# BattleZips/BattleZips-Halo2

Hardware: AMD Instinct MI355X
Metric: complete proofs per second (synthesis + create_proof), BoardCircuit, k=14, IPA/Pasta (higher is better)
Workload: dtype u32x8 (255-bit modular integer, Montgomery)

## Files before the change

### battlezips-halo2_amd/csrc/ntt.hip

```cpp
#include <cstdlib>
#include <cstring>
#include <vector>

#include "ntt_common.cuh"

namespace bzh {

template <class P>
void launch_ntt_pass_wave(const NttPassArgs& aa, unsigned tiles, unsigned nb, hipStream_t stream);
extern template void launch_ntt_pass_wave<FpParams>(const NttPassArgs&, unsigned, unsigned, hipStream_t);
extern template void launch_ntt_pass_wave<FqParams>(const NttPassArgs&, unsigned, unsigned, hipStream_t);
extern template void launch_ntt_pass_wave<BnFrParams>(const NttPassArgs&, unsigned, unsigned, hipStream_t);

template <class P, int C, bool FIRST>
__device__ __forceinline__ void stage_group(uint4* tile, const NttPassArgs& g, int s0, int items, int tid) {
    constexpr int E = 1 << C;
    const int r = g.r, logW = g.logW, W = 1 << logW;
    const int ngroups = items >> C;
    const int stride = 1 << (s0 + logW);
    for (int gi = tid; gi < ngroups; gi += kNttThreads) {
        const int col = gi & (W - 1), gg = gi >> logW;
        const int lo = gg & ((1 << s0) - 1), hi = gg >> s0;
        const int base = ((((hi << C) << s0) | lo) << logW) + col;
        Fe<P> x[E];
#pragma unroll
        for (int m = 0; m < E; m++) x[m] = tile_get<P>(tile, base + m * stride);
#pragma unroll
        for (int t = 0; t < C; t++) {
            const int sh = r - 1 - (s0 + t);
#pragma unroll
            for (int b = 0; b < E / 2; b++) {
                const int jm = b & ((1 << t) - 1), top = ((b >> t) << (t + 1)) + jm, bot = top + (1 << t);
                Fe<P> v = x[bot];
                if (!(FIRST && jm == 0)) {
                    const int j = FIRST ? jm : (lo | (jm << s0));
                    v = fe_mul(v, fe_load<P>(g.sub_tw + ((size_t)j << sh) * 8));
                }
                x[bot] = fe_sub(x[top], v);
                x[top] = fe_add(x[top], v);
            }
            __builtin_amdgcn_sched_barrier(0);
        }
#pragma unroll
        for (int m = 0; m < E; m++) tile_put(tile, base + m * stride, x[m]);
    }
}

template <class P>
__global__ void __launch_bounds__(kNttThreads) __attribute__((amdgpu_waves_per_eu(2))) k_ntt_pass(NttPassArgs g) {
    __shared__ __align__(16) uint4 tile[2 * kTileElems];
    const int tid = threadIdx.x, T = kNttThreads;
    const int r = g.r, R = 1 << r, logW = g.logW, W = 1 << logW;
    const size_t N = (size_t)1 << g.log_n;
    const uint32_t* vin = g.src + (size_t)blockIdx.y * N * 8;
    uint32_t* vec = g.dst + (size_t)blockIdx.y * N * 8;
    const size_t tile_id = blockIdx.x;
    const int items = R << logW;

    if (!g.last) {
        const size_t B = (size_t)1 << g.logB;
        const size_t tiles_per_a = B >> logW;
        const size_t a = tile_id / tiles_per_a, j0 = (tile_id - a * tiles_per_a) << logW;
        const uint32_t* base = vin + ((a << (r + g.logB)) + j0) * 8;
        if (g.nz) {
            const uint32_t* sv = g.src + (size_t)blockIdx.y * (N >> g.nz) * 8 + j0 * 8;
            const int live = items >> g.nz;
            for (int it = tid; it < live; it += T) {
                const int col = it & (W - 1), row = it >> logW;
                Fe<P> v = fe_load<P>(sv + ((size_t)row * B + col) * 8);
                if (g.pre_lo) v = fe_mul(v, pow_table<P>(g.pre_lo, g.pre_hi, g.h, (size_t)row * B + j0 + col));
                if (g.cube_pre) {
                    const unsigned c3 = (unsigned)(((size_t)row * B + j0 + col) % 3);
                    if (c3) v = fe_mul(v, cube_const<P>(g, c3));
                }
                const int p0 = (int)(bitrev((uint32_t)row, r) << logW) + col;
                for (int m = 0; m < (1 << g.nz); m++) tile_put(tile, p0 + (m << logW), v);
            }
        } else
        for (int it = tid; it < items; it += T) {
            const int col = it & (W - 1), row = it >> logW;
            Fe<P> v = fe_load<P>(base + ((size_t)row * B + col) * 8);
            if (g.pre_lo) v = fe_mul(v, pow_table<P>(g.pre_lo, g.pre_hi, g.h, (size_t)row * B + j0 + col));
            if (g.cube_pre) {
                const unsigned c3 = (unsigned)(((size_t)row * B + j0 + col) % 3);
                if (c3) v = fe_mul(v, cube_const<P>(g, c3));
            }
            tile_put(tile, (int)(bitrev((uint32_t)row, r) << logW) + col, v);
        }
    } else {
        for (int it = tid; it < items; it += T) {
            const int rr = it & (R - 1), i = it >> r;
            size_t d = (tile_id << logW) + i, a = 0;
            for (int q = 0; q < g.nprev; q++) {
                a = (a << g.prev_bits[q]) | (d & (((size_t)1 << g.prev_bits[q]) - 1));
                d >>= g.prev_bits[q];
            }
            Fe<P> v = fe_load<P>(vin + ((a << r) + rr) * 8);
            if (g.pre_lo) v = fe_mul(v, pow_table<P>(g.pre_lo, g.pre_hi, g.h, (size_t)rr));
            if (g.cube_pre && (rr % 3)) v = fe_mul(v, cube_const<P>(g, (unsigned)(rr % 3)));
            tile_put(tile, (int)(bitrev((uint32_t)rr, r) << logW) + i, v);
        }
    }
    {
        int s0 = g.nz ? g.nz : (r < 3 ? r : 3);
        if (!g.nz) {
            __syncthreads();
            switch (s0) {
                case 1: stage_group<P, 1, true>(tile, g, 0, items, tid); break;
                case 2: stage_group<P, 2, true>(tile, g, 0, items, tid); break;
                default: stage_group<P, 3, true>(tile, g, 0, items, tid); break;
            }
        }
        int ngr = (r - s0 + 2) / 3;
        for (; ngr > 0; ngr--) {
            const int c = (r - s0 + ngr - 1) / ngr;
            __syncthreads();
            switch (c) {
                case 1: stage_group<P, 1, false>(tile, g, s0, items, tid); break;
                case 2: stage_group<P, 2, false>(tile, g, s0, items, tid); break;
                default: stage_group<P, 3, false>(tile, g, s0, items, tid); break;
            }
            s0 += c;
        }
    }
    __syncthreads();
    if (!g.last) {
        const size_t B = (size_t)1 << g.logB;
        const size_t tiles_per_a = B >> logW;
        const size_t a = tile_id / tiles_per_a, j0 = (tile_id - a * tiles_per_a) << logW;
        uint32_t* base = vec + ((a << (r + g.logB)) + j0) * 8;
        for (int it = tid; it < items; it += T) {
            const int col = it & (W - 1), row = it >> logW;
            Fe<P> v = tile_get<P>(tile, it);
            if (g.tw_direct) {
                v = fe_mul(v, fe_load<P>(g.tw_direct + ((size_t)row * B + j0 + col) * 8));
            } else {
                const size_t e = ((size_t)row * (j0 + col)) << g.logA;
                if (e || g.tw_always) v = fe_mul(v, pow_table<P>(g.tw_lo, g.tw_hi, g.h, e));
            }
            fe_store(base + ((size_t)row * B + col) * 8, v);
        }
    } else {
        for (int it = tid; it < items; it += T) {
            const int i = it & (W - 1), kr = it >> logW;
            Fe<P> v = tile_get<P>(tile, it);
            const size_t k = ((size_t)kr << g.logA) + (tile_id << logW) + i;
            if (g.post_lo) v = fe_mul(v, pow_table<P>(g.post_lo, g.post_hi, g.h, k));
            if (g.cube_post) v = fe_mul(v, cube_const<P>(g, (unsigned)(k % 3)));
            ntt_store_out<P>(g, vec, (size_t)blockIdx.y, (size_t)1 << g.log_n, k, v);
        }
    }
}

struct NttDomain {
    int field;
    unsigned log_n;
    int inverse;
    int has_shift;
    uint32_t omega[8];
    uint32_t shift[8];
    int h;
    uint32_t* d_tables = nullptr;
    size_t off_tw_lo, off_tw_hi, off_sc_lo, off_sc_hi;
    size_t off_tw_hi_scaled;
    int shift_is_cube;
    uint32_t cube[3][8];
    size_t off_sub[12];
    size_t off_direct[4];
};

struct NttCache {
    std::vector<NttDomain> doms;
};
static std::mutex g_cache_mu;
static std::vector<std::pair<bzh_ctx*, NttCache*>> g_caches;

static NttCache* cache_for(bzh_ctx* ctx) {
    std::lock_guard<std::mutex> lk(g_cache_mu);
    for (auto& p : g_caches)
        if (p.first == ctx) return p.second;
    g_caches.emplace_back(ctx, new NttCache());
    return g_caches.back().second;
}
void ntt_cache_drop(bzh_ctx* ctx) {
    std::lock_guard<std::mutex> lk(g_cache_mu);
    for (size_t i = 0; i < g_caches.size(); i++)
        if (g_caches[i].first == ctx) {
            for (auto& d : g_caches[i].second->doms)
                if (d.d_tables) (void)hipFree(d.d_tables);
            delete g_caches[i].second;
            g_caches.erase(g_caches.begin() + i);
            return;
        }
}

template <class P>
static void fill_pows(std::vector<uint32_t>& out, size_t off, const Fe<P>& base, const Fe<P>& first, size_t count) {
    Fe<P> acc = first;
    for (size_t i = 0; i < count; i++) {
        for (int k = 0; k < 8; k++) out[off + i * 8 + k] = acc.l[k];
        acc = fe_mul(acc, base);
    }
}
template <class P>
static Fe<P> pow2k(Fe<P> x, int k) {
    for (int i = 0; i < k; i++) x = fe_sqr(x);
    return x;
}

static int plan_passes(unsigned log_n, int* bits) {
    if (log_n <= 11) {
        bits[0] = (int)log_n;
        return 1;
    }
    const int np = (int)((log_n + 8) / 9);
    const int base = (int)log_n / np, extra = (int)log_n % np;
    for (int i = 0; i < np; i++) bits[i] = base + (i < extra ? 1 : 0);
    return np;
}
static constexpr unsigned kDirectTwiddleMaxLog = 20;

template <class P>
static int build_domain(bzh_ctx* ctx, NttDomain& d, const Fe<P>& omega_m, const Fe<P>* shift_m) {
    const unsigned k = d.log_n;
    const size_t N = (size_t)1 << k;
    d.h = (int)((k + 1) / 2);
    const size_t nlo = (size_t)1 << d.h, nhi = (size_t)1 << (k - d.h);
    Fe<P> w = d.inverse ? fe_inv(omega_m) : omega_m;
    size_t words = 0;
    d.off_tw_lo = words; words += nlo * 8;
    d.off_tw_hi = words; words += nhi * 8;
    d.off_sc_lo = words; words += nlo * 8;
    d.off_sc_hi = words; words += nhi * 8;
    d.off_tw_hi_scaled = words; words += nhi * 8;
    for (int rb = 1; rb <= 11; rb++) {
        d.off_sub[rb] = words;
        if ((unsigned)rb <= k) words += ((size_t)1 << (rb - 1)) * 8;
    }
    int bits[5];
    const int np = plan_passes(k, bits);
    for (int p = 0; p < 4; p++) d.off_direct[p] = 0;
    if (np >= 2 && k <= kDirectTwiddleMaxLog) {
        int logA = 0;
        for (int p = 0; p + 1 < np; p++) {
            d.off_direct[p] = words;
            words += (N >> logA) * 8;
            logA += bits[p];
        }
    }
    std::vector<uint32_t> host(words, 0u);
    fill_pows<P>(host, d.off_tw_lo, w, fe_one<P>(), nlo);
    fill_pows<P>(host, d.off_tw_hi, pow2k(w, d.h), fe_one<P>(), nhi);
    Fe<P> sbase = fe_one<P>(), first_hi = fe_one<P>();
    if (d.has_shift) sbase = d.inverse ? fe_inv(*shift_m) : *shift_m;
    if (d.inverse) {
        Fe<P> nn = fe_zero<P>();
        nn.l[0] = (uint32_t)(N & 0xffffffffu);
        nn.l[1] = (uint32_t)((uint64_t)N >> 32);
        first_hi = fe_inv(fe_to_mont(nn));
    }
    fill_pows<P>(host, d.off_sc_lo, sbase, fe_one<P>(), nlo);
    fill_pows<P>(host, d.off_sc_hi, pow2k(sbase, d.h), first_hi, nhi);
    fill_pows<P>(host, d.off_tw_hi_scaled, pow2k(w, d.h), first_hi, nhi);
    {
        const Fe<P> s2 = fe_sqr(sbase), s3 = fe_mul(s2, sbase);
        d.shift_is_cube = d.has_shift && fe_eq(s3, fe_one<P>()) && !fe_eq(sbase, fe_one<P>());
        const Fe<P> c0 = first_hi, c1 = fe_mul(first_hi, sbase), c2 = fe_mul(first_hi, s2);
        for (int q = 0; q < 8; q++) {
            d.cube[0][q] = c0.l[q];
            d.cube[1][q] = c1.l[q];
            d.cube[2][q] = c2.l[q];
        }
    }
    for (int rb = 1; rb <= 11 && (unsigned)rb <= k; rb++) {
        Fe<P> wr = pow2k(w, (int)k - rb);
        fill_pows<P>(host, d.off_sub[rb], wr, fe_one<P>(), (size_t)1 << (rb - 1));
    }
    if (d.off_direct[0]) {
        int logA = 0;
        for (int p = 0; p + 1 < np; p++) {
            const size_t R = (size_t)1 << bits[p], B = N >> (logA + bits[p]);
            const Fe<P> wa = pow2k(w, logA);
            const Fe<P> first = (p == 0 && d.inverse && !d.has_shift) ? first_hi : fe_one<P>();
            Fe<P> wrow = fe_one<P>();
            for (size_t row = 0; row < R; row++) {
                fill_pows<P>(host, d.off_direct[p] + row * B * 8, wrow, first, B);
                wrow = fe_mul(wrow, wa);
            }
            logA += bits[p];
        }
    }
    BZH_HIP_TRY(ctx, hipMalloc((void**)&d.d_tables, words * 4));
    BZH_HIP_TRY(ctx, hipMemcpyAsync(d.d_tables, host.data(), words * 4, hipMemcpyHostToDevice, ctx->stream));
    BZH_HIP_TRY(ctx, hipStreamSynchronize(ctx->stream));
    return BZH_OK;
}

template <class P>
static int ntt_run_t(bzh_ctx* ctx, uint32_t* d_data, unsigned log_n, size_t batch, const uint64_t* omega,
                     const uint64_t* coset_shift, int inverse, int form, const uint32_t* d_src = nullptr, unsigned src_log = 0,
                     uint32_t* d_out29 = nullptr) {
    if (log_n == 0) return d_out29 ? BZH_E_ARG : BZH_OK;
    Fe<P> w, sh = fe_one<P>();
    for (int i = 0; i < 4; i++) {
        w.l[2 * i] = (uint32_t)omega[i];
        w.l[2 * i + 1] = (uint32_t)(omega[i] >> 32);
        if (coset_shift) {
            sh.l[2 * i] = (uint32_t)coset_shift[i];
            sh.l[2 * i + 1] = (uint32_t)(coset_shift[i] >> 32);
        }
    }
    if (form == BZH_FORM_CANONICAL) {
        w = fe_to_mont(w);
        if (coset_shift) sh = fe_to_mont(sh);
    }
    NttCache* cache = cache_for(ctx);
    NttDomain* dom = nullptr;
    for (auto& d : cache->doms) {
        if (d.field == P::id && d.log_n == log_n && d.inverse == (inverse != 0) && d.has_shift == (coset_shift != nullptr) &&
            memcmp(d.omega, w.l, 32) == 0 && (!coset_shift || memcmp(d.shift, sh.l, 32) == 0)) {
            dom = &d;
            break;
        }
    }
    if (!dom) {
        NttDomain d;
        d.field = P::id;
        d.log_n = log_n;
        d.inverse = inverse != 0;
        d.has_shift = coset_shift != nullptr;
        memcpy(d.omega, w.l, 32);
        memcpy(d.shift, sh.l, 32);
        int rc = build_domain<P>(ctx, d, w, coset_shift ? &sh : nullptr);
        if (rc) return rc;
        cache->doms.push_back(d);
        dom = &cache->doms.back();
    }
    const size_t total = batch << log_n;
    if (form == BZH_FORM_CANONICAL) {
        int rc = field_convert(ctx, P::id, d_data, total, 1);
        if (rc) return rc;
    }
    int bits[5];
    const int np = plan_passes(log_n, bits);
    int nz = 0;
    if (d_src) {
        if (src_log > log_n || form != BZH_FORM_MONTGOMERY) return BZH_E_ARG;
        nz = (int)(log_n - src_log);
        if ((np < 2 || nz > bits[0] || nz == 0) && !d_data) return BZH_E_ARG;
        if (np < 2 || nz > bits[0] || nz == 0) {
            BZH_HIP_TRY(ctx, hipMemsetAsync(d_data, 0, total * 32, ctx->stream));
            BZH_HIP_TRY(ctx, hipMemcpy2DAsync(d_data, ((size_t)32) << log_n, d_src, ((size_t)32) << src_log, ((size_t)32) << src_log, batch,
                                              hipMemcpyDeviceToDevice, ctx->stream));
            nz = 0;
            d_src = nullptr;
        }
    }
    uint32_t* d_scratch = nullptr;
    if (np >= 2) {
        void* sp = nullptr;
        int rc = ws_ensure(ctx, 0, total * 32, &sp);
        if (rc) return rc;
        d_scratch = (uint32_t*)sp;
    }
    const bool pre = (!inverse && coset_shift);
    const bool post = (inverse != 0);
    int logA = 0;
    for (int p = 0; p < np; p++) {
        NttPassArgs a;
        a.src = (p == 0) ? (nz ? d_src : d_data) : d_scratch;
        a.nz = (p == 0) ? nz : 0;
        a.dst = (p == np - 1) ? d_data : d_scratch;
        a.log_n = log_n;
        a.r = bits[p];
        a.logA = logA;
        a.logB = (int)log_n - logA - bits[p];
        a.last = (p == np - 1);
        int logW = 11 - a.r;
        if (!a.last && logW > a.logB) logW = a.logB;
        if (a.last && logW > logA) logW = logA;
        a.logW = logW;
        a.nprev = p;
        for (int q = 0; q < 4; q++) a.prev_bits[q] = q < p ? bits[q] : 0;
        a.sub_tw = dom->d_tables + dom->off_sub[a.r];
        a.tw_lo = dom->d_tables + dom->off_tw_lo;
        a.tw_hi = dom->d_tables + dom->off_tw_hi;
        a.tw_direct = (p + 1 < np && dom->off_direct[p]) ? dom->d_tables + dom->off_direct[p] : nullptr;
        a.h = dom->h;
        a.pre_lo = (pre && p == 0) ? dom->d_tables + dom->off_sc_lo : nullptr;
        a.pre_hi = dom->d_tables + dom->off_sc_hi;
        a.post_lo = (post && a.last) ? dom->d_tables + dom->off_sc_lo : nullptr;
        a.post_hi = dom->d_tables + dom->off_sc_hi;
        a.cube_pre = a.cube_post = a.tw_always = 0;
        a.dst29 = nullptr;
        memcpy(a.cube, dom->cube, sizeof(a.cube));
        if (pre && dom->shift_is_cube) {
            if (p == 0) a.cube_pre = 1;
            a.pre_lo = nullptr;
        }
        if (post) {
            if (coset_shift && dom->shift_is_cube) {
                a.post_lo = nullptr;
                a.cube_post = a.last ? 1 : 0;
            } else if (!coset_shift) {
                a.post_lo = nullptr;
                if (np == 1) {
                    a.cube_post = 1;
                } else if (p == 0) {
                    a.tw_hi = dom->d_tables + dom->off_tw_hi_scaled;
                    a.tw_always = 1;
                }
            }
        }
        const size_t tiles = ((size_t)1 << log_n) >> (a.r + logW);
        {
            ScopedTimer t(ctx, BZH_T_NTT);
            if (ctx->profiling && p == 0)
                ctx->alg_bytes[BZH_T_NTT] += (32.0 + (nz ? 32.0 / (double)(1 << nz) : 32.0)) * (double)batch * (double)((size_t)1 << log_n);
            for (size_t b0 = 0; b0 < batch; b0 += 65535) {
                size_t nb = batch - b0 < 65535 ? batch - b0 : 65535;
                NttPassArgs aa = a;
                aa.src = a.src + (b0 << (log_n - (unsigned)a.nz)) * 8;
                aa.dst = a.dst ? a.dst + (b0 << log_n) * 8 : nullptr;
                aa.dst29 = (a.last && d_out29) ? d_out29 + (b0 << log_n) * 9 : nullptr;
                static const bool lds_only = getenv("BZH_NTT_LDS") != nullptr;
                const dim3 grid((unsigned)tiles, (unsigned)nb), blk(kNttThreads);
                constexpr bool wave_ok = P::id != BZH_FIELD_BN254_FQ;
                if (wave_ok && !lds_only && a.r >= 6 && a.r <= 9 && logW == 11 - a.r && a.nz <= 3) {
                    if constexpr (wave_ok) launch_ntt_pass_wave<P>(aa, (unsigned)tiles, (unsigned)nb, ctx->stream);
                } else {
                    hipLaunchKernelGGL((k_ntt_pass<P>), grid, blk, 0, ctx->stream, aa);
                }
            }
        }
        BZH_HIP_TRY(ctx, hipGetLastError());
        logA += bits[p];
    }
    if (form == BZH_FORM_CANONICAL) {
        int rc = field_convert(ctx, P::id, d_data, total, 0);
        if (rc) return rc;
    }
    return BZH_OK;
}

template <class P>
__global__ void __launch_bounds__(256) k_field_convert(uint32_t* data, size_t count, int to_mont) {
    size_t gid = blockIdx.x * (size_t)blockDim.x + threadIdx.x;
    if (gid >= count) return;
    Fe<P> v = fe_load<P>(data + gid * 8);
    fe_store(data + gid * 8, to_mont ? fe_to_mont(v) : fe_from_mont(v));
}

int field_convert(bzh_ctx* ctx, int field, uint32_t* d, size_t count, int to_mont) {
    if (!count) return BZH_OK;
    dim3 grid((unsigned)((count + 255) / 256)), block(256);
    switch (field) {
        case BZH_FIELD_FP: hipLaunchKernelGGL((k_field_convert<FpParams>), grid, block, 0, ctx->stream, d, count, to_mont); break;
        case BZH_FIELD_FQ: hipLaunchKernelGGL((k_field_convert<FqParams>), grid, block, 0, ctx->stream, d, count, to_mont); break;
        case BZH_FIELD_BN254_FR: hipLaunchKernelGGL((k_field_convert<BnFrParams>), grid, block, 0, ctx->stream, d, count, to_mont); break;
        case BZH_FIELD_BN254_FQ: hipLaunchKernelGGL((k_field_convert<BnFqParams>), grid, block, 0, ctx->stream, d, count, to_mont); break;
        default: return BZH_E_ARG;
    }
    BZH_HIP_TRY(ctx, hipGetLastError());
    return BZH_OK;
}

int ntt_run(bzh_ctx* ctx, int field, uint32_t* d_data, unsigned log_n, size_t batch, const uint64_t* omega,
            const uint64_t* coset_shift, int inverse, int form) {
    switch (field) {
        case BZH_FIELD_FP: return ntt_run_t<FpParams>(ctx, d_data, log_n, batch, omega, coset_shift, inverse, form);
        case BZH_FIELD_FQ: return ntt_run_t<FqParams>(ctx, d_data, log_n, batch, omega, coset_shift, inverse, form);
        case BZH_FIELD_BN254_FR: return ntt_run_t<BnFrParams>(ctx, d_data, log_n, batch, omega, coset_shift, inverse, form);
        case BZH_FIELD_BN254_FQ: return ntt_run_t<BnFqParams>(ctx, d_data, log_n, batch, omega, coset_shift, inverse, form);
    }
    return BZH_E_ARG;
}

int ntt_run_padded(bzh_ctx* ctx, int field, uint32_t* d_dst, const uint32_t* d_src, unsigned src_log, unsigned log_n, size_t batch,
                   const uint64_t* omega, const uint64_t* coset_shift, uint32_t* d_out29) {
    const int f = BZH_FORM_MONTGOMERY;
    if (d_out29 && field != BZH_FIELD_FP && field != BZH_FIELD_FQ) return BZH_E_ARG;
    switch (field) {
        case BZH_FIELD_FP: return ntt_run_t<FpParams>(ctx, d_dst, log_n, batch, omega, coset_shift, 0, f, d_src, src_log, d_out29);
        case BZH_FIELD_FQ: return ntt_run_t<FqParams>(ctx, d_dst, log_n, batch, omega, coset_shift, 0, f, d_src, src_log, d_out29);
        case BZH_FIELD_BN254_FR: return ntt_run_t<BnFrParams>(ctx, d_dst, log_n, batch, omega, coset_shift, 0, f, d_src, src_log);
        case BZH_FIELD_BN254_FQ: return ntt_run_t<BnFqParams>(ctx, d_dst, log_n, batch, omega, coset_shift, 0, f, d_src, src_log);
    }
    return BZH_E_ARG;
}

}
```

### battlezips-halo2_amd/csrc/ntt_common.cuh

```cuda
#pragma once
#include "ctx.hpp"
#include "field.cuh"
#include "fe29.cuh"

namespace bzh {

static constexpr int kTileElems = 2048;
static constexpr int kNttThreads = 256;

struct NttPassArgs {
    const uint32_t* src;
    uint32_t* dst;
    unsigned log_n;
    int r;
    int logA;
    int logB;
    int logW;
    int last;
    int nprev;
    int prev_bits[4];
    const uint32_t* sub_tw;
    const uint32_t* tw_lo;
    const uint32_t* tw_hi;
    const uint32_t* tw_direct;
    int h;
    const uint32_t* pre_lo;
    const uint32_t* pre_hi;
    const uint32_t* post_lo;
    const uint32_t* post_hi;
    int cube_pre;
    int cube_post;
    int tw_always;
    int nz;
    uint32_t cube[3][8];
    uint32_t* dst29;
};
template <class P>
__device__ __forceinline__ void ntt_store_out(const NttPassArgs& g, uint32_t* vec, size_t vec_index, size_t N, size_t k, const Fe<P>& v) {
    if constexpr (fe29_supported<P>()) {
        if (g.dst29) {
            fe29_store_planes<P>(g.dst29 + vec_index * 9 * N, k, N, fe29_from_sat_reduced(v));
            return;
        }
    }
    fe_store(vec + k * 8, v);
}

template <class P>
__device__ __forceinline__ Fe<P> tile_get(const uint4* t, int idx) {
    uint4 a = t[idx], b = t[kTileElems + idx];
    Fe<P> r;
    r.l[0] = a.x; r.l[1] = a.y; r.l[2] = a.z; r.l[3] = a.w;
    r.l[4] = b.x; r.l[5] = b.y; r.l[6] = b.z; r.l[7] = b.w;
    return r;
}
template <class P>
__device__ __forceinline__ void tile_put(uint4* t, int idx, const Fe<P>& v) {
    t[idx] = make_uint4(v.l[0], v.l[1], v.l[2], v.l[3]);
    t[kTileElems + idx] = make_uint4(v.l[4], v.l[5], v.l[6], v.l[7]);
}
template <class P>
__device__ __forceinline__ Fe<P> pow_table(const uint32_t* lo, const uint32_t* hi, int h, size_t e) {
    Fe<P> a = fe_load<P>(lo + (e & (((size_t)1 << h) - 1)) * 8);
    Fe<P> b = fe_load<P>(hi + (e >> h) * 8);
    return fe_mul(a, b);
}
template <class P>
__device__ __forceinline__ Fe<P> cube_const(const NttPassArgs& g, unsigned i) {
    Fe<P> r;
#pragma unroll
    for (int k = 0; k < 8; k++) r.l[k] = i == 0 ? g.cube[0][k] : (i == 1 ? g.cube[1][k] : g.cube[2][k]);
    return r;
}
__device__ __forceinline__ uint32_t bitrev(uint32_t x, int bits) { return bits ? (__brev(x) >> (32 - bits)) : 0u; }


}
```

### battlezips-halo2_amd/csrc/ntt_wave.cuh

```cuda
#pragma once
#include "ntt_common.cuh"

namespace bzh {

template <int LB>
__device__ __forceinline__ void lane_swap_u32(uint32_t& lo, uint32_t& hi, bool lane_bit) {
    if constexpr (LB == 5) {
        auto r = __builtin_amdgcn_permlane32_swap(lo, hi, false, false);
        lo = r[0], hi = r[1];
    } else if constexpr (LB == 4) {
        auto r = __builtin_amdgcn_permlane16_swap(lo, hi, false, false);
        lo = r[0], hi = r[1];
    } else if constexpr (LB == 3) {
        const uint32_t nh = (uint32_t)__builtin_amdgcn_update_dpp((int)hi, (int)lo, 0x108 , 0xf, 0x3, false);
        const uint32_t nl = (uint32_t)__builtin_amdgcn_update_dpp((int)lo, (int)hi, 0x118 , 0xf, 0xc, false);
        lo = nl, hi = nh;
    } else if constexpr (LB == 2) {
        const uint32_t nh = (uint32_t)__builtin_amdgcn_update_dpp((int)hi, (int)lo, 0x104 , 0xf, 0x5, false);
        const uint32_t nl = (uint32_t)__builtin_amdgcn_update_dpp((int)lo, (int)hi, 0x114 , 0xf, 0xa, false);
        lo = nl, hi = nh;
    } else {
        const uint32_t send = lane_bit ? lo : hi;
        const uint32_t recv = (uint32_t)__builtin_amdgcn_mov_dpp((int)send, LB == 1 ? 0x4e  : 0xb1 ,
                                                                 0xf, 0xf, false);
        lo = lane_bit ? recv : lo;
        hi = lane_bit ? hi : recv;
    }
}
template <class P, int RB, int LB>
__device__ __forceinline__ void lane_swap(Fe<P> (&x)[8], int lane) {
    const bool lb = (lane >> LB) & 1;
#pragma unroll
    for (int m = 0; m < 8; m++) {
        if (m & (1 << RB)) continue;
#pragma unroll
        for (int q = 0; q < 8; q++) lane_swap_u32<LB>(x[m].l[q], x[m | (1 << RB)].l[q], lb);
    }
}
template <class P, int RB, class Tw>
__device__ __forceinline__ void reg_stage(Fe<P> (&x)[8], Tw tw) {
#pragma unroll
    for (int m = 0; m < 8; m++) {
        if (m & (1 << RB)) continue;
        Fe<P> v = x[m | (1 << RB)];
        const uint32_t* t = tw(m);
        if (t) v = fe_mul(v, fe_load<P>(t));
        x[m | (1 << RB)] = fe_sub(x[m], v);
        x[m] = fe_add(x[m], v);
    }
    __builtin_amdgcn_sched_barrier(0);
}

template <class P, int R, bool LAST>
__global__ void __launch_bounds__(kNttThreads) k_ntt_pass_wave(NttPassArgs g) {
    static_assert(R >= 6 && R <= 9, "three register bits + three to six lane bits");
    constexpr int RL = R - 3, CL = 6 - RL, N2 = RL - 3;
    const int lane = threadIdx.x & 63, wave = threadIdx.x >> 6;
    const int logW = g.logW;
    const int col = (wave << CL) | (lane & ((1 << CL) - 1));
    const int lr = lane >> CL;
    const size_t N = (size_t)1 << g.log_n;
    const uint32_t* vin = g.src + (size_t)blockIdx.y * N * 8;
    uint32_t* vec = g.dst + (size_t)blockIdx.y * N * 8;
    const size_t tile_id = blockIdx.x;
    const size_t B = (size_t)1 << g.logB;
    const size_t tiles_per_a = LAST ? 1 : (B >> logW);
    const size_t a_idx = LAST ? 0 : tile_id / tiles_per_a, j0 = LAST ? 0 : ((tile_id - a_idx * tiles_per_a) << logW);

    Fe<P> x[8];
    if (!LAST) {
        const uint32_t* base = g.nz ? g.src + (size_t)blockIdx.y * (N >> g.nz) * 8 + j0 * 8 : vin + ((a_idx << (R + g.logB)) + j0) * 8;
        const int rep = g.nz ? (1 << g.nz) : 1;
#pragma unroll
        for (int m = 0; m < 8; m++) {
            if (m & (rep - 1)) continue;
            const uint32_t t = ((uint32_t)lr << 3) | (uint32_t)m;
            const size_t row = bitrev(t, R);
            Fe<P> v = fe_load<P>(base + (row * B + col) * 8);
            if (g.pre_lo) v = fe_mul(v, pow_table<P>(g.pre_lo, g.pre_hi, g.h, row * B + j0 + col));
            if (g.cube_pre) {
                const unsigned c3 = (unsigned)((row * B + j0 + col) % 3);
                if (c3) v = fe_mul(v, cube_const<P>(g, c3));
            }
            x[m] = v;
        }
        if (g.nz >= 1) x[1] = x[0], x[3] = x[2], x[5] = x[4], x[7] = x[6];
        if (g.nz >= 2) x[2] = x[0], x[3] = x[0], x[6] = x[4], x[7] = x[4];
        if (g.nz >= 3) x[4] = x[0], x[5] = x[0], x[6] = x[0], x[7] = x[0];
    } else {
        size_t d = (tile_id << logW) + col, a = 0;
        for (int q = 0; q < g.nprev; q++) {
            a = (a << g.prev_bits[q]) | (d & (((size_t)1 << g.prev_bits[q]) - 1));
            d >>= g.prev_bits[q];
        }
#pragma unroll
        for (int m = 0; m < 8; m++) {
            const uint32_t t = ((uint32_t)lr << 3) | (uint32_t)m;
            const size_t rr = bitrev(t, R);
            Fe<P> v = fe_load<P>(vin + ((a << R) + rr) * 8);
            if (g.pre_lo) v = fe_mul(v, pow_table<P>(g.pre_lo, g.pre_hi, g.h, rr));
            if (g.cube_pre && (rr % 3)) v = fe_mul(v, cube_const<P>(g, (unsigned)(rr % 3)));
            x[m] = v;
        }
    }
    const uint32_t* sub = g.sub_tw;
    if (g.nz < 1) reg_stage<P, 0>(x, [&](int) -> const uint32_t* { return nullptr; });
    if (g.nz < 2) reg_stage<P, 1>(x, [&](int m) -> const uint32_t* { return (m & 1) ? sub + ((size_t)(m & 1) << (R - 2)) * 8 : nullptr; });
    if (g.nz < 3) reg_stage<P, 2>(x, [&](int m) -> const uint32_t* { return (m & 3) ? sub + ((size_t)(m & 3) << (R - 3)) * 8 : nullptr; });
    lane_swap<P, 0, CL + 0>(x, lane);
    lane_swap<P, 1, CL + 1>(x, lane);
    lane_swap<P, 2, CL + 2>(x, lane);
    const uint32_t lo3 = (uint32_t)(lane >> CL) & 7u;
    reg_stage<P, 0>(x, [&](int) -> const uint32_t* { return sub + ((size_t)lo3 << (R - 4)) * 8; });
    reg_stage<P, 1>(x, [&](int m) -> const uint32_t* { return sub + ((size_t)(lo3 | ((uint32_t)(m & 1) << 3)) << (R - 5)) * 8; });
    reg_stage<P, 2>(x, [&](int m) -> const uint32_t* { return sub + ((size_t)(lo3 | ((uint32_t)(m & 3) << 3)) << (R - 6)) * 8; });
    if constexpr (N2 >= 1) lane_swap<P, 0, (N2 >= 1 ? CL + 3 : 0)>(x, lane);
    if constexpr (N2 >= 2) lane_swap<P, 1, (N2 >= 2 ? CL + 4 : 0)>(x, lane);
    if constexpr (N2 >= 3) lane_swap<P, 2, (N2 >= 3 ? CL + 5 : 0)>(x, lane);
    const uint32_t mid_lane = N2 ? (((uint32_t)lane >> (CL + 3)) & ((1u << N2) - 1u)) : 0u;
    auto mid3 = [&](int m) -> uint32_t { return mid_lane | ((uint32_t)m & (7u & ~((1u << N2) - 1u))); };
    if constexpr (N2 >= 1) reg_stage<P, 0>(x, [&](int m) -> const uint32_t* { return sub + ((size_t)(lo3 | (mid3(m) << 3)) << (R - 7)) * 8; });
    if constexpr (N2 >= 2)
        reg_stage<P, 1>(x, [&](int m) -> const uint32_t* { return sub + ((size_t)(lo3 | (mid3(m) << 3) | ((uint32_t)(m & 1) << 6)) << (R - 8)) * 8; });
    if constexpr (N2 >= 3)
        reg_stage<P, 2>(x, [&](int m) -> const uint32_t* { return sub + ((size_t)(lo3 | (mid3(m) << 3) | ((uint32_t)(m & 3) << 6)) << (R - 9)) * 8; });
#pragma unroll
    for (int m = 0; m < 8; m++) {
        const uint32_t t = lo3 | (mid3(m) << 3) | (((uint32_t)m & ((1u << N2) - 1u)) << 6);
        Fe<P> v = x[m];
        if (!LAST) {
            uint32_t* base = vec + ((a_idx << (R + g.logB)) + j0) * 8;
            if (g.tw_direct) {
                v = fe_mul(v, fe_load<P>(g.tw_direct + ((size_t)t * B + j0 + col) * 8));
            } else {
                const size_t e = ((size_t)t * (j0 + col)) << g.logA;
                if (e || g.tw_always) v = fe_mul(v, pow_table<P>(g.tw_lo, g.tw_hi, g.h, e));
            }
            fe_store(base + ((size_t)t * B + col) * 8, v);
        } else {
            const size_t k = ((size_t)t << g.logA) + (tile_id << logW) + col;
            if (g.post_lo) v = fe_mul(v, pow_table<P>(g.post_lo, g.post_hi, g.h, k));
            if (g.cube_post) v = fe_mul(v, cube_const<P>(g, (unsigned)(k % 3)));
            ntt_store_out<P>(g, vec, (size_t)blockIdx.y, N, k, v);
        }
    }
}


template <class P>
void launch_ntt_pass_wave(const NttPassArgs& aa, unsigned tiles, unsigned nb, hipStream_t stream) {
    const dim3 grid(tiles, nb), blk(kNttThreads);
#define BZH_WAVE_PASS(RB)                                                                          \
    if (aa.last) hipLaunchKernelGGL((k_ntt_pass_wave<P, RB, true>), grid, blk, 0, stream, aa);      \
    else hipLaunchKernelGGL((k_ntt_pass_wave<P, RB, false>), grid, blk, 0, stream, aa)
    switch (aa.r) {
        case 6: BZH_WAVE_PASS(6); break;
        case 7: BZH_WAVE_PASS(7); break;
        case 8: BZH_WAVE_PASS(8); break;
        default: BZH_WAVE_PASS(9); break;
    }
#undef BZH_WAVE_PASS
}

}
```

### battlezips-halo2_amd/csrc/ntt_wave_fp.hip

```cpp
#include "ntt_wave.cuh"
namespace bzh {
template void launch_ntt_pass_wave<FpParams>(const NttPassArgs&, unsigned, unsigned, hipStream_t);
}
```

### battlezips-halo2_amd/csrc/ntt_wave_fq.hip

```cpp
#include "ntt_wave.cuh"
namespace bzh {
template void launch_ntt_pass_wave<FqParams>(const NttPassArgs&, unsigned, unsigned, hipStream_t);
}
```

Before: 731.5.

## Run multi-pass wave NTT in lazy 29-bit limb representation with planar intermediates

Adds a wave-shuffle NTT kernel that keeps field elements in a 9×29-bit redundant limb form with compile-time bound tracking. Carries and folds are inserted only where the computed bounds require them. Intermediates between passes are stored in a planar 9-limb layout, and separate 29-bit twiddle tables are built at domain setup. The aim is to cut Montgomery reduction and carry work per butterfly, at the cost of larger scratch traffic (36 vs 32 bytes per element), extra table memory, and more complex correctness reasoning.

```diff
diff --git a/battlezips-halo2_amd/csrc/ntt.hip b/battlezips-halo2_amd/csrc/ntt.hip
--- a/battlezips-halo2_amd/csrc/ntt.hip
+++ b/battlezips-halo2_amd/csrc/ntt.hip
@@ -11,6 +11,10 @@
 extern template void launch_ntt_pass_wave<FpParams>(const NttPassArgs&, unsigned, unsigned, hipStream_t);
 extern template void launch_ntt_pass_wave<FqParams>(const NttPassArgs&, unsigned, unsigned, hipStream_t);
 extern template void launch_ntt_pass_wave<BnFrParams>(const NttPassArgs&, unsigned, unsigned, hipStream_t);
+template <class P>
+void launch_ntt_pass_wave29(const NttPassArgs& aa, unsigned tiles, unsigned nb, hipStream_t stream);
+extern template void launch_ntt_pass_wave29<FpParams>(const NttPassArgs&, unsigned, unsigned, hipStream_t);
+extern template void launch_ntt_pass_wave29<FqParams>(const NttPassArgs&, unsigned, unsigned, hipStream_t);
 
 template <class P, int C, bool FIRST>
 __device__ __forceinline__ void stage_group(uint4* tile, const NttPassArgs& g, int s0, int items, int tid) {
@@ -167,6 +171,11 @@
     uint32_t cube[3][8];
     size_t off_sub[12];
     size_t off_direct[4];
+    uint32_t* d_tables29 = nullptr;
+    size_t off29_tw_lo, off29_tw_hi, off29_sc_lo, off29_sc_hi, off29_tw_hi_scaled;
+    size_t off29_sub[12];
+    size_t off29_direct[4];
+    uint32_t cube29[3][9];
 };
 
 struct NttCache {
@@ -186,8 +195,10 @@
     std::lock_guard<std::mutex> lk(g_cache_mu);
     for (size_t i = 0; i < g_caches.size(); i++)
         if (g_caches[i].first == ctx) {
-            for (auto& d : g_caches[i].second->doms)
+            for (auto& d : g_caches[i].second->doms) {
                 if (d.d_tables) (void)hipFree(d.d_tables);
+                if (d.d_tables29) (void)hipFree(d.d_tables29);
+            }
             delete g_caches[i].second;
             g_caches.erase(g_caches.begin() + i);
             return;
@@ -208,16 +219,6 @@
     return x;
 }
 
-static int plan_passes(unsigned log_n, int* bits) {
-    if (log_n <= 11) {
-        bits[0] = (int)log_n;
-        return 1;
-    }
-    const int np = (int)((log_n + 8) / 9);
-    const int base = (int)log_n / np, extra = (int)log_n % np;
-    for (int i = 0; i < np; i++) bits[i] = base + (i < extra ? 1 : 0);
-    return np;
-}
 static constexpr unsigned kDirectTwiddleMaxLog = 20;
 
 template <class P>
@@ -292,6 +293,68 @@
     }
     BZH_HIP_TRY(ctx, hipMalloc((void**)&d.d_tables, words * 4));
     BZH_HIP_TRY(ctx, hipMemcpyAsync(d.d_tables, host.data(), words * 4, hipMemcpyHostToDevice, ctx->stream));
+    if constexpr (fe29_supported<P>()) {
+        if (np >= 2) {
+            auto to29 = [](const uint32_t* v8) {
+                Fe<P> v;
+                for (int q = 0; q < 8; q++) v.l[q] = v8[q];
+                for (int q = 0; q < 5; q++) v = fe_add(v, v);
+                return fe29_from_raw<P>(v.l);
+            };
+            size_t w29 = 0;
+            auto seg = [&](size_t count) { const size_t o = w29; w29 += count * 12; return o; };
+            d.off29_tw_lo = seg(nlo);
+            d.off29_tw_hi = seg(nhi);
+            d.off29_sc_lo = seg(nlo);
+            d.off29_sc_hi = seg(nhi);
+            d.off29_tw_hi_scaled = seg(nhi);
+            for (int rb = 1; rb <= 11; rb++) d.off29_sub[rb] = seg((unsigned)rb <= k ? (size_t)1 << (rb - 1) : 0);
+            for (int p = 0; p < 4; p++) d.off29_direct[p] = 0;
+            if (d.off_direct[0]) {
+                int logA = 0;
+                for (int p = 0; p + 1 < np; p++) {
+                    d.off29_direct[p] = w29;
+                    w29 += (N >> logA) * 9;
+                    logA += bits[p];
+                }
+            }
+            std::vector<uint32_t> h29(w29, 0u);
+            auto copy = [&](size_t off, size_t off29, size_t count) {
+                for (size_t i = 0; i < count; i++) {
+                    const Fe29<P> v = to29(&host[off + i * 8]);
+                    for (int q = 0; q < 9; q++) h29[off29 + i * 12 + q] = v.l[q];
+                }
+            };
+            copy(d.off_tw_lo, d.off29_tw_lo, nlo);
+            copy(d.off_tw_hi, d.off29_tw_hi, nhi);
+            copy(d.off_sc_lo, d.off29_sc_lo, nlo);
+            copy(d.off_sc_hi, d.off29_sc_hi, nhi);
+            copy(d.off_tw_hi_scaled, d.off29_tw_hi_scaled, nhi);
+            for (int rb = 1; rb <= 11 && (unsigned)rb <= k; rb++) copy(d.off_sub[rb], d.off29_sub[rb], (size_t)1 << (rb - 1));
+            if (d.off_direct[0]) {
+                int logA = 0;
+                for (int p = 0; p + 1 < np; p++) {
+                    const size_t M = N >> logA, o = d.off29_direct[p];
+                    for (size_t i = 0; i < M; i++) {
+                        const Fe29<P> v = to29(&host[d.off_direct[p] + i * 8]);
+                        for (int q = 0; q < 4; q++) {
+                            h29[o + i * 4 + q] = v.l[q];
+                            h29[o + 4 * M + i * 4 + q] = v.l[4 + q];
+                        }
+                        h29[o + 8 * M + i] = v.l[8];
+                    }
+                    logA += bits[p];
+                }
+            }
+            for (int c = 0; c < 3; c++) {
+                const Fe29<P> v = to29(d.cube[c]);
+                for (int q = 0; q < 9; q++) d.cube29[c][q] = v.l[q];
+            }
+            BZH_HIP_TRY(ctx, hipStreamSynchronize(ctx->stream));
+            BZH_HIP_TRY(ctx, hipMalloc((void**)&d.d_tables29, w29 * 4));
+            BZH_HIP_TRY(ctx, hipMemcpyAsync(d.d_tables29, h29.data(), w29 * 4, hipMemcpyHostToDevice, ctx->stream));
+        }
+    }
     BZH_HIP_TRY(ctx, hipStreamSynchronize(ctx->stream));
     return BZH_OK;
 }
@@ -356,10 +419,24 @@
             d_src = nullptr;
         }
     }
+    static const bool lds_only = getenv("BZH_NTT_LDS") != nullptr;
+    constexpr bool wave_ok = P::id != BZH_FIELD_BN254_FQ;
+    auto pass_logW = [&](int p, int logA) {
+        int logW = 11 - bits[p];
+        const int logB = (int)log_n - logA - bits[p];
+        if (p + 1 < np && logW > logB) logW = logB;
+        if (p + 1 == np && logW > logA) logW = logA;
+        return logW;
+    };
+    auto pass_wave = [&](int p, int logA) {
+        return wave_ok && !lds_only && bits[p] >= 6 && bits[p] <= 9 && pass_logW(p, logA) == 11 - bits[p] && (p ? 0 : nz) <= 3;
+    };
+    bool use29 = fe29_supported<P>() && np >= 2 && dom->d_tables29 != nullptr;
+    for (int p = 0, logA = 0; p < np && use29; logA += bits[p], p++) use29 = pass_wave(p, logA);
     uint32_t* d_scratch = nullptr;
     if (np >= 2) {
         void* sp = nullptr;
-        int rc = ws_ensure(ctx, 0, total * 32, &sp);
+        int rc = ws_ensure(ctx, 0, total * (use29 ? 36 : 32), &sp);
         if (rc) return rc;
         d_scratch = (uint32_t*)sp;
     }
@@ -376,9 +453,7 @@
         a.logA = logA;
         a.logB = (int)log_n - logA - bits[p];
         a.last = (p == np - 1);
-        int logW = 11 - a.r;
-        if (!a.last && logW > a.logB) logW = a.logB;
-        if (a.last && logW > logA) logW = logA;
+        const int logW = pass_logW(p, logA);
         a.logW = logW;
         a.nprev = p;
         for (int q = 0; q < 4; q++) a.prev_bits[q] = q < p ? bits[q] : 0;
@@ -394,6 +469,7 @@
         a.cube_pre = a.cube_post = a.tw_always = 0;
         a.dst29 = nullptr;
         memcpy(a.cube, dom->cube, sizeof(a.cube));
+        memcpy(a.cube29, dom->cube29, sizeof(a.cube29));
         if (pre && dom->shift_is_cube) {
             if (p == 0) a.cube_pre = 1;
             a.pre_lo = nullptr;
@@ -412,6 +488,17 @@
                 }
             }
         }
+        if (use29) {
+            const uint32_t* t29 = dom->d_tables29;
+            a.sub_tw = t29 + dom->off29_sub[a.r];
+            a.tw_lo = t29 + dom->off29_tw_lo;
+            a.tw_hi = t29 + (a.tw_hi == dom->d_tables + dom->off_tw_hi_scaled ? dom->off29_tw_hi_scaled : dom->off29_tw_hi);
+            a.tw_direct = a.tw_direct ? t29 + dom->off29_direct[p] : nullptr;
+            a.pre_lo = a.pre_lo ? t29 + dom->off29_sc_lo : nullptr;
+            a.pre_hi = t29 + dom->off29_sc_hi;
+            a.post_lo = a.post_lo ? t29 + dom->off29_sc_lo : nullptr;
+            a.post_hi = t29 + dom->off29_sc_hi;
+        }
         const size_t tiles = ((size_t)1 << log_n) >> (a.r + logW);
         {
             ScopedTimer t(ctx, BZH_T_NTT);
@@ -420,13 +507,17 @@
             for (size_t b0 = 0; b0 < batch; b0 += 65535) {
                 size_t nb = batch - b0 < 65535 ? batch - b0 : 65535;
                 NttPassArgs aa = a;
-                aa.src = a.src + (b0 << (log_n - (unsigned)a.nz)) * 8;
-                aa.dst = a.dst ? a.dst + (b0 << log_n) * 8 : nullptr;
+                aa.src = a.src + (b0 << (log_n - (unsigned)a.nz)) * (use29 && p > 0 ? 9 : 8);
+                aa.dst = a.dst ? a.dst + (b0 << log_n) * (use29 && !a.last ? 9 : 8) : nullptr;
                 aa.dst29 = (a.last && d_out29) ? d_out29 + (b0 << log_n) * 9 : nullptr;
-                static const bool lds_only = getenv("BZH_NTT_LDS") != nullptr;
                 const dim3 grid((unsigned)tiles, (unsigned)nb), blk(kNttThreads);
-                constexpr bool wave_ok = P::id != BZH_FIELD_BN254_FQ;
-                if (wave_ok && !lds_only && a.r >= 6 && a.r <= 9 && logW == 11 - a.r && a.nz <= 3) {
+                if constexpr (fe29_supported<P>()) {
+                    if (use29) {
+                        launch_ntt_pass_wave29<P>(aa, (unsigned)tiles, (unsigned)nb, ctx->stream);
+                        continue;
+                    }
+                }
+                if (pass_wave(p, logA)) {
                     if constexpr (wave_ok) launch_ntt_pass_wave<P>(aa, (unsigned)tiles, (unsigned)nb, ctx->stream);
                 } else {
                     hipLaunchKernelGGL((k_ntt_pass<P>), grid, blk, 0, ctx->stream, aa);
diff --git a/battlezips-halo2_amd/csrc/ntt_common.cuh b/battlezips-halo2_amd/csrc/ntt_common.cuh
--- a/battlezips-halo2_amd/csrc/ntt_common.cuh
+++ b/battlezips-halo2_amd/csrc/ntt_common.cuh
@@ -34,7 +34,152 @@
     int nz;
     uint32_t cube[3][8];
     uint32_t* dst29;
-};
+    uint32_t cube29[3][9];
+};
+
+inline int plan_passes(unsigned log_n, int* bits) {
+    if (log_n <= 11) {
+        bits[0] = (int)log_n;
+        return 1;
+    }
+    const int np = (int)((log_n + 8) / 9);
+    const int base = (int)log_n / np, extra = (int)log_n % np;
+    for (int i = 0; i < np; i++) bits[i] = base + (i < extra ? 1 : 0);
+    return np;
+}
+
+struct Ntt29Bnd {
+    uint32_t v;
+    uint64_t l;
+    uint64_t l8;
+};
+constexpr uint64_t kN29LimbMax = 0xffffffffull;
+constexpr uint64_t kN29MulLimb = 3ull << 30;
+constexpr uint32_t kN29MulV = 127;
+constexpr uint32_t kN29MulVAny = 63;
+constexpr uint64_t kN29BiasLimb = (3ull << 29) - 1;
+constexpr uint64_t kN29Carried = (1ull << 29) + 8, kN29Carried8 = (1ull << 23) + 16;
+enum { kN29Carry = 1, kN29Fold = 2, kN29Exact = 4 };
+enum { kN29StageNone = 0, kN29StageSome = 1, kN29StageAll = 2 };
+enum { kN29NextStage = 0, kN29NextMul = 1, kN29NextOut = 2 };
+
+constexpr Ntt29Bnd ntt29_entry() { return Ntt29Bnd{2, kN29Carried, kN29Carried8}; }
+constexpr Ntt29Bnd ntt29_product() { return Ntt29Bnd{2, (1ull << 29) - 1, 1ull << 23}; }
+constexpr uint64_t ntt29_max(uint64_t a, uint64_t b) { return a > b ? a : b; }
+constexpr Ntt29Bnd ntt29_join(Ntt29Bnd a, Ntt29Bnd b) { return Ntt29Bnd{a.v > b.v ? a.v : b.v, ntt29_max(a.l, b.l), ntt29_max(a.l8, b.l8)}; }
+constexpr bool ntt29_le(Ntt29Bnd a, Ntt29Bnd b) { return a.v <= b.v && a.l <= b.l && a.l8 <= b.l8; }
+constexpr bool ntt29_mul_ok(Ntt29Bnd b) { return b.l <= kN29MulLimb && b.l8 <= kN29MulLimb && b.v <= kN29MulV; }
+constexpr int ntt29_k_plain(Ntt29Bnd b) {
+    int K = 4;
+    while (K < 128 && ((uint64_t)K << 22) - 2 < b.l8) K *= 2;
+    return K;
+}
+struct Ntt29Step {
+    bool ok;
+    Ntt29Bnd a, b;
+    int K;
+};
+constexpr Ntt29Step ntt29_stage(Ntt29Bnd s, int kind) {
+    Ntt29Step r{true, s, s, 4};
+    if (kind != kN29StageNone) {
+        r.ok = r.ok && ntt29_mul_ok(s);
+        const Ntt29Bnd t = ntt29_product();
+        r.a = Ntt29Bnd{s.v + t.v, s.l + t.l, s.l8 + t.l8};
+        r.b = Ntt29Bnd{s.v + 4, s.l + kN29BiasLimb, s.l8 + (4ull << 22)};
+    }
+    if (kind != kN29StageAll) {
+        r.K = ntt29_k_plain(s);
+        r.ok = r.ok && s.l <= (1ull << 30) - 2 && ((uint64_t)r.K << 22) - 2 >= s.l8;
+        const Ntt29Bnd a{2 * s.v, 2 * s.l, 2 * s.l8}, b{s.v + (uint32_t)r.K, s.l + kN29BiasLimb, s.l8 + ((uint64_t)r.K << 22)};
+        r.a = kind == kN29StageNone ? a : ntt29_join(r.a, a);
+        r.b = kind == kN29StageNone ? b : ntt29_join(r.b, b);
+    }
+    r.ok = r.ok && r.a.l <= kN29LimbMax && r.a.l8 <= kN29LimbMax && r.b.l <= kN29LimbMax && r.b.l8 <= kN29LimbMax;
+    return r;
+}
+constexpr Ntt29Bnd ntt29_carry(Ntt29Bnd s) {
+    return Ntt29Bnd{s.v, kN29Carried, s.l8 + 8};
+}
+constexpr bool ntt29_fold_ok(Ntt29Bnd s) { return s.l + kN29BiasLimb <= kN29LimbMax && s.l8 < (1ull << 29); }
+constexpr Ntt29Bnd ntt29_fold(Ntt29Bnd) { return Ntt29Bnd{3, kN29Carried, (1ull << 23) + 8}; }
+constexpr bool ntt29_admits(Ntt29Bnd s, int next, int kind) {
+    if (next == kN29NextStage) {
+        const Ntt29Step st = ntt29_stage(s, kind);
+        return st.ok && st.a.l8 < (1ull << 29) && st.b.l8 < (1ull << 29) && st.a.v <= 127 && st.b.v <= 127;
+    }
+    const bool mul = ntt29_mul_ok(s) && s.v <= kN29MulVAny;
+    if (next == kN29NextMul) return mul;
+    return mul && s.l <= kN29LimbMax - 8 && s.l8 <= kN29LimbMax - 8;
+}
+constexpr int ntt29_fix_for(Ntt29Bnd s, int next, int kind) {
+    if (ntt29_admits(s, next, kind)) return 0;
+    if (ntt29_admits(ntt29_carry(s), next, kind)) return kN29Carry;
+    if (ntt29_fold_ok(s) && ntt29_admits(ntt29_fold(s), next, kind)) return kN29Fold;
+    if (ntt29_fold_ok(ntt29_carry(s)) && ntt29_admits(ntt29_fold(s), next, kind)) return kN29Carry | kN29Fold;
+    return -1;
+}
+constexpr Ntt29Bnd ntt29_apply(Ntt29Bnd s, int fix) {
+    if (fix & kN29Carry) s = ntt29_carry(s);
+    if (fix & kN29Fold) s = ntt29_fold(s);
+    return s;
+}
+constexpr int ntt29_stage_kind(int s) { return s == 0 ? kN29StageNone : (s < 3 ? kN29StageSome : kN29StageAll); }
+
+struct Ntt29Plan {
+    bool ok;
+    int K[9];
+    int fix_a[9], fix_b[9];
+    Ntt29Bnd in[10];
+    int leaf_fix;
+};
+constexpr Ntt29Plan ntt29_plan(int R, bool last) {
+    Ntt29Plan p{};
+    p.ok = R >= 1 && R <= 9;
+    Ntt29Bnd s = ntt29_entry();
+    for (int i = 0; i < R && p.ok; i++) {
+        p.in[i] = s;
+        const Ntt29Step st = ntt29_stage(s, ntt29_stage_kind(i));
+        p.ok = st.ok;
+        p.K[i] = st.K;
+        const int next = i + 1 < R ? kN29NextStage : (last ? kN29NextOut : kN29NextMul);
+        const int kind = i + 1 < R ? ntt29_stage_kind(i + 1) : 0;
+        p.fix_a[i] = ntt29_fix_for(st.a, next, kind);
+        p.fix_b[i] = ntt29_fix_for(st.b, next, kind);
+        p.ok = p.ok && p.fix_a[i] >= 0 && p.fix_b[i] >= 0;
+        if (p.ok) s = ntt29_join(ntt29_apply(st.a, p.fix_a[i]), ntt29_apply(st.b, p.fix_b[i]));
+    }
+    p.in[R] = s;
+    const Ntt29Bnd leaf{2, kN29Carried, kN29Carried8};
+    p.leaf_fix = ntt29_le(s, leaf) ? 0 : (kN29Exact | kN29Fold);
+    return p;
+}
+
+template <class P>
+BZH_HD Fe29<P> ntt29_carry_exact(const Fe29<P>& a) {
+    Fe29<P> r;
+    uint32_t c = 0;
+#pragma unroll
+    for (int i = 0; i < 8; i++) {
+        const uint32_t t = a.l[i] + c;
+        r.l[i] = t & kM29;
+        c = t >> 29;
+    }
+    r.l[8] = a.l[8] + c;
+    return r;
+}
+template <class P, int FIX>
+BZH_HD Fe29<P> ntt29_fix(Fe29<P> x) {
+    if constexpr ((FIX & kN29Exact) != 0) x = ntt29_carry_exact(x);
+    if constexpr ((FIX & kN29Carry) != 0) x = fe29_carry(x);
+    if constexpr ((FIX & kN29Fold) != 0) x = fe29_fold(x);
+    return x;
+}
+template <class P, bool W, int K, int FA, int FB>
+BZH_HD void ntt29_butterfly(Fe29<P>& a, Fe29<P>& b, const Fe29<P>& w) {
+    const Fe29<P> t = W ? fe29_mul(w, b) : b;
+    b = ntt29_fix<P, FB>(fe29_sub_lazy<P, (W ? 4 : K), 1>(a, t));
+    a = ntt29_fix<P, FA>(fe29_add(a, t));
+}
 template <class P>
 __device__ __forceinline__ void ntt_store_out(const NttPassArgs& g, uint32_t* vec, size_t vec_index, size_t N, size_t k, const Fe<P>& v) {
     if constexpr (fe29_supported<P>()) {
diff --git a/battlezips-halo2_amd/csrc/ntt_wave.cuh b/battlezips-halo2_amd/csrc/ntt_wave.cuh
--- a/battlezips-halo2_amd/csrc/ntt_wave.cuh
+++ b/battlezips-halo2_amd/csrc/ntt_wave.cuh
@@ -147,6 +147,146 @@
 }
 
 
+template <class P, int RB, int LB>
+__device__ __forceinline__ void lane_swap29(Fe29<P> (&x)[8], int lane) {
+    const bool lb = (lane >> LB) & 1;
+#pragma unroll
+    for (int m = 0; m < 8; m++) {
+        if (m & (1 << RB)) continue;
+#pragma unroll
+        for (int q = 0; q < 9; q++) lane_swap_u32<LB>(x[m].l[q], x[m | (1 << RB)].l[q], lb);
+    }
+}
+template <class P, int RB, int K, int FA, int FB, class Tw>
+__device__ __forceinline__ void reg_stage29(Fe29<P> (&x)[8], Tw tw) {
+    static_for<8>([&](auto mi) {
+        constexpr int m = decltype(mi)::value;
+        if constexpr ((m & (1 << RB)) == 0) {
+            const uint32_t* t = tw(m);
+            if (t) ntt29_butterfly<P, true, K, FA, FB>(x[m], x[m | (1 << RB)], fe29_load_const<P>(t));
+            else ntt29_butterfly<P, false, K, FA, FB>(x[m], x[m | (1 << RB)], x[m]);
+        }
+    });
+    __builtin_amdgcn_sched_barrier(0);
+}
+#define BZH_STAGE29(S, RB, TW) reg_stage29<P, RB, PL.K[S], PL.fix_a[S], PL.fix_b[S]>(x, TW)
+template <class P>
+__device__ __forceinline__ Fe29<P> pow_table29(const uint32_t* lo, const uint32_t* hi, int h, size_t e) {
+    return fe29_mul(fe29_load_const<P>(lo + (e & (((size_t)1 << h) - 1)) * 12), fe29_load_const<P>(hi + (e >> h) * 12));
+}
+template <class P>
+__device__ __forceinline__ Fe29<P> cube29_const(const NttPassArgs& g, unsigned i) {
+    Fe29<P> r;
+#pragma unroll
+    for (int k = 0; k < 9; k++) r.l[k] = i == 0 ? g.cube29[0][k] : (i == 1 ? g.cube29[1][k] : g.cube29[2][k]);
+    return r;
+}
+
+template <class P, int R, bool LAST>
+__global__ void __launch_bounds__(kNttThreads) k_ntt_pass_wave29(NttPassArgs g) {
+    static_assert(R >= 6 && R <= 9, "three register bits + three to six lane bits");
+    constexpr Ntt29Plan PL = ntt29_plan(R, LAST);
+    static_assert(PL.ok, "fe29 NTT: no bound schedule for this pass");
+    constexpr int RL = R - 3, CL = 6 - RL, N2 = RL - 3;
+    const int lane = threadIdx.x & 63, wave = threadIdx.x >> 6;
+    const int logW = g.logW;
+    const int col = (wave << CL) | (lane & ((1 << CL) - 1));
+    const int lr = lane >> CL;
+    const size_t N = (size_t)1 << g.log_n;
+    const size_t tile_id = blockIdx.x;
+    const size_t B = (size_t)1 << g.logB;
+    const size_t tiles_per_a = LAST ? 1 : (B >> logW);
+    const size_t a_idx = LAST ? 0 : tile_id / tiles_per_a, j0 = LAST ? 0 : ((tile_id - a_idx * tiles_per_a) << logW);
+
+    Fe29<P> x[8];
+    if (!LAST) {
+        const size_t base = (a_idx << (R + g.logB)) + j0;
+        if (g.nprev == 0) {
+            const uint32_t* src = g.nz ? g.src + (size_t)blockIdx.y * (N >> g.nz) * 8 + j0 * 8 : g.src + ((size_t)blockIdx.y * N + base) * 8;
+            const int rep = g.nz ? (1 << g.nz) : 1;
+            static_for<8>([&](auto mi) {
+                constexpr int m = decltype(mi)::value;
+                if (m & (rep - 1)) return;
+                const uint32_t t = ((uint32_t)lr << 3) | (uint32_t)m;
+                const size_t row = bitrev(t, R);
+                Fe29<P> v = fe29_from_sat_reduced(fe_load<P>(src + (row * B + col) * 8));
+                if (g.pre_lo) v = fe29_mul(v, pow_table29<P>(g.pre_lo, g.pre_hi, g.h, row * B + j0 + col));
+                if (g.cube_pre) {
+                    const unsigned c3 = (unsigned)((row * B + j0 + col) % 3);
+                    if (c3) v = fe29_mul(v, cube29_const<P>(g, c3));
+                }
+                x[m] = v;
+            });
+            if (g.nz >= 1) x[1] = x[0], x[3] = x[2], x[5] = x[4], x[7] = x[6];
+            if (g.nz >= 2) x[2] = x[0], x[3] = x[0], x[6] = x[4], x[7] = x[4];
+            if (g.nz >= 3) x[4] = x[0], x[5] = x[0], x[6] = x[0], x[7] = x[0];
+        } else {
+            const uint32_t* src = g.src + (size_t)blockIdx.y * N * 9;
+            static_for<8>([&](auto mi) {
+                constexpr int m = decltype(mi)::value;
+                const uint32_t t = ((uint32_t)lr << 3) | (uint32_t)m;
+                x[m] = fe29_load_planes<P>(src, base + bitrev(t, R) * B + col, N);
+            });
+        }
+    } else {
+        size_t d = (tile_id << logW) + col, a = 0;
+        for (int q = 0; q < g.nprev; q++) {
+            a = (a << g.prev_bits[q]) | (d & (((size_t)1 << g.prev_bits[q]) - 1));
+            d >>= g.prev_bits[q];
+        }
+        const uint32_t* src = g.src + (size_t)blockIdx.y * N * 9;
+#pragma unroll
+        for (int m = 0; m < 8; m++) {
+            const uint32_t t = ((uint32_t)lr << 3) | (uint32_t)m;
+            x[m] = fe29_load_planes<P>(src, (a << R) + bitrev(t, R), N);
+        }
+    }
+    const uint32_t* sub = g.sub_tw;
+    if (g.nz < 1) BZH_STAGE29(0, 0, [&](int) -> const uint32_t* { return nullptr; });
+    if (g.nz < 2) BZH_STAGE29(1, 1, [&](int m) -> const uint32_t* { return (m & 1) ? sub + ((size_t)(m & 1) << (R - 2)) * 12 : nullptr; });
+    if (g.nz < 3) BZH_STAGE29(2, 2, [&](int m) -> const uint32_t* { return (m & 3) ? sub + ((size_t)(m & 3) << (R - 3)) * 12 : nullptr; });
+    lane_swap29<P, 0, CL + 0>(x, lane);
+    lane_swap29<P, 1, CL + 1>(x, lane);
+    lane_swap29<P, 2, CL + 2>(x, lane);
+    const uint32_t lo3 = (uint32_t)(lane >> CL) & 7u;
+    BZH_STAGE29(3, 0, [&](int) -> const uint32_t* { return sub + ((size_t)lo3 << (R - 4)) * 12; });
+    BZH_STAGE29(4, 1, [&](int m) -> const uint32_t* { return sub + ((size_t)(lo3 | ((uint32_t)(m & 1) << 3)) << (R - 5)) * 12; });
+    BZH_STAGE29(5, 2, [&](int m) -> const uint32_t* { return sub + ((size_t)(lo3 | ((uint32_t)(m & 3) << 3)) << (R - 6)) * 12; });
+    if constexpr (N2 >= 1) lane_swap29<P, 0, (N2 >= 1 ? CL + 3 : 0)>(x, lane);
+    if constexpr (N2 >= 2) lane_swap29<P, 1, (N2 >= 2 ? CL + 4 : 0)>(x, lane);
+    if constexpr (N2 >= 3) lane_swap29<P, 2, (N2 >= 3 ? CL + 5 : 0)>(x, lane);
+    const uint32_t mid_lane = N2 ? (((uint32_t)lane >> (CL + 3)) & ((1u << N2) - 1u)) : 0u;
+    auto mid3 = [&](int m) -> uint32_t { return mid_lane | ((uint32_t)m & (7u & ~((1u << N2) - 1u))); };
+    if constexpr (N2 >= 1) BZH_STAGE29((N2 >= 1 ? 6 : 0), 0, [&](int m) -> const uint32_t* { return sub + ((size_t)(lo3 | (mid3(m) << 3)) << (R - 7)) * 12; });
+    if constexpr (N2 >= 2)
+        BZH_STAGE29((N2 >= 2 ? 7 : 0), 1, [&](int m) -> const uint32_t* { return sub + ((size_t)(lo3 | (mid3(m) << 3) | ((uint32_t)(m & 1) << 6)) << (R - 8)) * 12; });
+    if constexpr (N2 >= 3)
+        BZH_STAGE29((N2 >= 3 ? 8 : 0), 2, [&](int m) -> const uint32_t* { return sub + ((size_t)(lo3 | (mid3(m) << 3) | ((uint32_t)(m & 3) << 6)) << (R - 9)) * 12; });
+    static_for<8>([&](auto mi) {
+        constexpr int m = decltype(mi)::value;
+        const uint32_t t = lo3 | (mid3(m) << 3) | (((uint32_t)m & ((1u << N2) - 1u)) << 6);
+        Fe29<P> v = x[m];
+        if (!LAST) {
+            if (g.tw_direct) v = fe29_mul(v, fe29_load_planes<P>(g.tw_direct, (size_t)t * B + j0 + col, (size_t)1 << (R + g.logB)));
+            else v = fe29_mul(v, pow_table29<P>(g.tw_lo, g.tw_hi, g.h, ((size_t)t * (j0 + col)) << g.logA));
+            fe29_store_planes<P>(g.dst + (size_t)blockIdx.y * N * 9, (a_idx << (R + g.logB)) + j0 + (size_t)t * B + col, N, v);
+        } else {
+            const size_t k = ((size_t)t << g.logA) + (tile_id << logW) + col;
+            bool scaled = false;
+            if (g.post_lo) v = fe29_mul(v, pow_table29<P>(g.post_lo, g.post_hi, g.h, k)), scaled = true;
+            if (g.cube_post) v = fe29_mul(v, cube29_const<P>(g, (unsigned)(k % 3))), scaled = true;
+            if (g.dst29) {
+                if (!scaled) v = ntt29_fix<P, PL.leaf_fix>(v);
+                fe29_store_planes<P>(g.dst29 + (size_t)blockIdx.y * 9 * N, k, N, v);
+            } else {
+                fe_store(g.dst + ((size_t)blockIdx.y * N + k) * 8, fe29_to_sat_div32(v));
+            }
+        }
+    });
+}
+#undef BZH_STAGE29
+
+
 template <class P>
 void launch_ntt_pass_wave(const NttPassArgs& aa, unsigned tiles, unsigned nb, hipStream_t stream) {
     const dim3 grid(tiles, nb), blk(kNttThreads);
@@ -161,5 +301,19 @@
     }
 #undef BZH_WAVE_PASS
 }
-
-}
+template <class P>
+void launch_ntt_pass_wave29(const NttPassArgs& aa, unsigned tiles, unsigned nb, hipStream_t stream) {
+    const dim3 grid(tiles, nb), blk(kNttThreads);
+#define BZH_WAVE_PASS(RB)                                                                            \
+    if (aa.last) hipLaunchKernelGGL((k_ntt_pass_wave29<P, RB, true>), grid, blk, 0, stream, aa);      \
+    else hipLaunchKernelGGL((k_ntt_pass_wave29<P, RB, false>), grid, blk, 0, stream, aa)
+    switch (aa.r) {
+        case 6: BZH_WAVE_PASS(6); break;
+        case 7: BZH_WAVE_PASS(7); break;
+        case 8: BZH_WAVE_PASS(8); break;
+        default: BZH_WAVE_PASS(9); break;
+    }
+#undef BZH_WAVE_PASS
+}
+
+}
diff --git a/battlezips-halo2_amd/csrc/ntt_wave_fp.hip b/battlezips-halo2_amd/csrc/ntt_wave_fp.hip
--- a/battlezips-halo2_amd/csrc/ntt_wave_fp.hip
+++ b/battlezips-halo2_amd/csrc/ntt_wave_fp.hip
@@ -1,4 +1,5 @@
 #include "ntt_wave.cuh"
 namespace bzh {
 template void launch_ntt_pass_wave<FpParams>(const NttPassArgs&, unsigned, unsigned, hipStream_t);
+template void launch_ntt_pass_wave29<FpParams>(const NttPassArgs&, unsigned, unsigned, hipStream_t);
 }
diff --git a/battlezips-halo2_amd/csrc/ntt_wave_fq.hip b/battlezips-halo2_amd/csrc/ntt_wave_fq.hip
--- a/battlezips-halo2_amd/csrc/ntt_wave_fq.hip
+++ b/battlezips-halo2_amd/csrc/ntt_wave_fq.hip
@@ -1,4 +1,5 @@
 #include "ntt_wave.cuh"
 namespace bzh {
 template void launch_ntt_pass_wave<FqParams>(const NttPassArgs&, unsigned, unsigned, hipStream_t);
+template void launch_ntt_pass_wave29<FqParams>(const NttPassArgs&, unsigned, unsigned, hipStream_t);
 }
```

After: 726.6, median of 2. No clear change (-0.7%).
